# samuel-watson/glmmrMCML

Measured on AMD Instinct MI355X. Metric: MCML iters/sec x m chains (simlik evals/sec), higher is better.
Workload: dtype f64

## Files before the change

### glmmrmcml_amd/api.py

```python
import ctypes as C
from contextlib import contextmanager as _contextmanager

import numpy as np

from . import _lib

c_dp = C.POINTER(C.c_double)
c_ip = C.POINTER(C.c_int32)

REDUCE_FN = C.CFUNCTYPE(C.c_int, C.c_void_p, C.c_void_p, C.c_int)


class Problem(C.Structure):
    _fields_ = [("cov", c_ip), ("cov_rows", C.c_int), ("data", c_dp), ("data_len", C.c_int),
                ("eff_range", c_dp), ("eff_len", C.c_int), ("Z", c_dp), ("X", c_dp), ("y", c_dp),
                ("n", C.c_int), ("Q", C.c_int), ("P", C.c_int), ("family", C.c_char_p),
                ("link", C.c_char_p)]


class DevOpts(C.Structure):
    _fields_ = [("device", C.c_int), ("stream", C.c_void_p), ("rank", C.c_int), ("world", C.c_int),
                ("reduce", REDUCE_FN), ("reduce_user", C.c_void_p)]


# ... 404 lines not shown
                                                       _p(out) if rows else None, rows, C.byref(n)))
        return out

    def last_kernels(self):
        names = {-1: None, 0: "skinny", 1: "band", 2: "dlds", 3: "reg", 4: "sparse", 5: "component", 6: "exact",
                 7: "exact_component"}
        f = C.c_int(); b = C.c_int()
        _lib.check(_lib.lib().glmmr_mcml_ctx_last_kernels(self._h, C.byref(f), C.byref(b)))
        return names[f.value], names[b.value]

    def band_plan(self, chains, which="fwd"):
        keys = ("used", "nbands", "tiles", "gn", "nwg", "nred", "nslots", "paired", "nempty", "built")
        return _plan(_lib.lib().glmmr_mcml_dbg_band_plan, C.c_int, keys, self._h, {"fwd": 0, "bwd": 1}[which], int(chains),
                     bools=("used", "paired", "built"))

    def sparse_plan(self, chains):
        keys = ("active", "factored", "W", "nnz", "nnz_z", "nnz_l", "nblk", "max_blk", "long_rows", "fused", "qrows", "ncb")
        return _plan(_lib.lib().glmmr_mcml_dbg_sparse_plan, C.c_longlong, keys, self._h, int(chains),
                     bools=("active", "factored", "long_rows"))

    def set_trajectory(self, mode):
        _TRAJ.set(self, mode)

    def component_plan(self, chains):
        keys = ("requested", "feasible", "used", "ncomp", "max_vars", "max_rows", "empty_comps", "nitems", "waves_per_item",
                "cap_vars", "lds_bytes_per_workgroup")
        return _plan(_lib.lib().glmmr_mcml_dbg_component_plan, C.c_longlong, keys, self._h, int(chains),
                     bools=("requested", "feasible", "used"))

    def set_draws(self, mode):
# ... 412 lines not shown
```

### glmmrmcml_amd/csrc/band_plan.h

```cpp
#pragma once
#include "common.h"
#include <algorithm>
#include <map>
#include <memory>

namespace mcml {

constexpr int BD_BM = 80, BD_BN = 128, BD_BK = 32, BD_STAGES = 3;
constexpr int BD_A_BYTES = BD_BK * BD_BM * 8;
constexpr int BD_B_BYTES = BD_BK * BD_BN * 8;
constexpr int BD_STAGE_BYTES = BD_A_BYTES + BD_B_BYTES;
constexpr size_t BD_LDS_BYTES = (size_t)BD_STAGES * BD_STAGE_BYTES;
constexpr int BD_NA = 3, BD_NB = 4, BD_PER_TILE = BD_NA + BD_NB;
constexpr int BD_TILE_ELEMS = BD_BM * BD_BN;

struct BandItem { int band, kt0, kt1, slot; };
struct BandRed { int band, s0, s1, pad; };

struct BandPlanDev {
    int gn = 0, nwg = 0, nred = 0, nslots = 0;
    int paired = 0;
    DevBuf items, wg_ptr, red, part;
};

struct SkinnyPlan {
    int nrb = 0, nkc = 0, ldp = 0;
    DevBuf range;
    DevBuf part;
};

struct BandPlan {
    int M = 0, K = 0, nbands = 0;
    std::vector<int> kr;
    long tiles = 0;
    std::map<int, std::unique_ptr<BandPlanDev>> by_gn;
    std::unique_ptr<SkinnyPlan> skinny;

    void reset(int M_, int K_, const std::vector<int>& kr_)
    {
        M = M_; K = K_; kr = kr_; nbands = (M + BD_BM - 1) / BD_BM;
        tiles = 0;
        for (int b = 0; b < nbands; ++b) tiles += kr[2 * b + 1] - kr[2 * b];
        by_gn.clear();
        skinny.reset();
    }

    static bool decompose(const std::vector<int>& kr, int nbands, int gn, int target_wg, std::vector<BandItem>& items,
                          std::vector<int>& wg_ptr, std::vector<BandRed>& red, int& nslots)
    {
        items.clear(); wg_ptr.clear(); red.clear(); nslots = 0;
        constexpr long OVH = 3;
        const int npairs = (nbands + 1) / 2;
        if ((long)npairs * gn * 5 >= (long)target_wg * 4) {
            auto cost = [&](int b) { return 2L * (kr[2 * b + 1] - kr[2 * b]) + OVH; };
            int G = target_wg / gn; if (G > nbands) G = nbands; if (G < 1) G = 1;
            std::vector<int> order(nbands);
            for (int b = 0; b < nbands; ++b) order[b] = b;
            std::stable_sort(order.begin(), order.end(), [&](int a, int b) { return cost(a) > cost(b); });
            std::vector<long> load(G, 0);
            std::vector<std::vector<int>> group(G);
// ... 54 lines not shown
        return false;
    }

    int device_plan(int gn, hipStream_t s, BandPlanDev** out)
    {
        auto it = by_gn.find(gn);
        if (it != by_gn.end()) { *out = it->second.get(); return MCML_OK; }
        std::unique_ptr<BandPlanDev> d(new BandPlanDev());
        std::vector<BandItem> items; std::vector<int> wg_ptr; std::vector<BandRed> red; int nslots = 0;
        d->paired = decompose(kr, nbands, gn, 256, items, wg_ptr, red, nslots) ? 1 : 0;
        d->gn = gn; d->nwg = (int)wg_ptr.size() - 1; d->nred = (int)red.size(); d->nslots = nslots;
        MCML_TRY(d->items.ensure(sizeof(BandItem) * (items.size() + 1)));
        MCML_TRY(d->wg_ptr.ensure(sizeof(int) * wg_ptr.size()));
        MCML_HIP(hipMemcpyAsync(d->items.p, items.data(), sizeof(BandItem) * items.size(), hipMemcpyHostToDevice, s));
        MCML_HIP(hipMemcpyAsync(d->wg_ptr.p, wg_ptr.data(), sizeof(int) * wg_ptr.size(), hipMemcpyHostToDevice, s));
        if (nslots > 0) {
            MCML_TRY(d->red.ensure(sizeof(BandRed) * red.size()));
            MCML_HIP(hipMemcpyAsync(d->red.p, red.data(), sizeof(BandRed) * red.size(), hipMemcpyHostToDevice, s));
            MCML_TRY(d->part.ensure(sizeof(double) * (size_t)nslots * gn * BD_TILE_ELEMS));
        }
        MCML_HIP(hipStreamSynchronize(s));
        *out = d.get();
        by_gn[gn] = std::move(d);
        return MCML_OK;
    }
};

}
```

### glmmrmcml_amd/csrc/cabi.hip

```cpp
#include "entry.h"
#include "hmc_chain.h"
#include <atomic>

using namespace mcml;

struct Mode {
    int Ctx::*field;
    const char* env;
    const char* names[4];
    const char* valid;
    std::atomic<int> dflt{-1};

    int get()
    {
        if (dflt.load() < 0) {
            const char* e = getenv(env);
            int unset = -1, m = 0;
            for (int i = 1; e && names[i]; ++i) if (!strcmp(e, names[i])) m = i;
            dflt.compare_exchange_strong(unset, m);
        }
        return dflt.load();
    }
    int check(const char* fn, bool ok, int mode) const
    {
// ... 360 lines not shown
{
    return m <= 0 ? 0 : sample_shape(m, 0, chains).ncols;
}

extern "C" int glmmr_mcml_ctx_profile(glmmr_mcml_ctx* h, int enable, int reset, double* out8)
{
    MCML_REQUIRE(h, "profile: null context");
    Ctx& c = h->c;
    KernelProf& p = c.prof;
    if (out8) {
        out8[0] = p.ms[0]; out8[1] = (double)p.cnt[0]; out8[2] = p.ms[1]; out8[3] = (double)p.cnt[1];
        const double C = (double)c.hmc.C, dense = 2.0 * c.n * (double)c.Q * C;
        double ff = dense, fb = dense, kind = 0;
        if (c.sp.active) { ff = fb = 2.0 * (double)c.sp.nnz * C; kind = 2; }
        else {
            if (c.band_fwd) { ff = 2.0 * 80.0 * 32.0 * (double)c.band_fwd_tiles * C; kind = 1; }
            if (c.band_bwd) { fb = 2.0 * 80.0 * 32.0 * (double)c.band_bwd_tiles * C; kind = 1; }
        }
        out8[4] = ff; out8[5] = fb; out8[6] = dense; out8[7] = kind;
    }
    if (reset) for (int i = 0; i < 4; ++i) { p.ms[i] = 0; p.cnt[i] = 0; p.seen[i] = 0; }
    if (enable && !p.on) {
        MCML_HIP(hipSetDevice(c.device));
        while (p.ev.size() < 4096) { hipEvent_t e; if (hipEventCreate(&e) != hipSuccess) { (void)hipGetLastError(); break; } p.ev.push_back(e); }
    }
    p.on = enable != 0;
    return MCML_OK;
}

extern "C" int glmmr_mcml_ctx_profile_launches(glmmr_mcml_ctx* h, long long* fwd, long long* bwd)
{
    MCML_REQUIRE(h, "profile_launches: null context");
// ... 354 lines not shown
```

### glmmrmcml_amd/csrc/ctx.h

```cpp
#pragma once
#include "common.h"
#include "chol.h"
#include "covspec.h"
#include "band_plan.h"
#include "component_plan.h"
#include "step_ahead.h"

namespace mcml {

typedef int (*reduce_fn)(void* user, double* dev_buf, int n);

enum { KERNEL_SKINNY = 0, KERNEL_BAND = 1, KERNEL_DLDS = 2, KERNEL_REG = 3, KERNEL_SPARSE = 4, KERNEL_COMPONENT = 5,
       KERNEL_EXACT = 6,
       KERNEL_EXACT_COMPONENT = 7 };

struct StepRing {
    static constexpr int SLOTS = StepAhead::SLOTS;
    unsigned long long* h = nullptr;
    unsigned long long* d = nullptr;
    unsigned seq = 0;
    StepRing() = default;
    StepRing(const StepRing&) = delete;
    StepRing& operator=(const StepRing&) = delete;
    ~StepRing() { if (h) (void)hipHostFree(h); }
// ... 148 lines not shown
    DevBuf y;
    DevBuf y_given;
    DevBuf d_cov, d_data, d_blocks, d_rowblock;

    DevMat U;
    int mcols = 0;
    int niter = 0;
    int m_global = 0, niter_global = 0;
    DevMat ZU;
    bool zu_valid = false;

    DevMat L, ZL, ZLT;
    BandPlan plan_fwd, plan_bwd;
    DevBuf kr_scratch;
    bool band_fwd = false, band_bwd = false;
    long band_fwd_tiles = 0, band_bwd_tiles = 0;
    DevBuf xb;
    bool have_L = false;

    DevMat Dwork;
    DevBuf partials;
    DevBuf scalars;
    int* errflag() const { return reinterpret_cast<int*>(scalars.d() + 16); }
    int maxdim_large = 0;
    int n_small = 0, n_diag_rows = 0;
    DevBuf small_ids;

    int last_kernel[2] = {-1, -1};
    HmcState hmc;
    NutsState nuts;
    KernelProf prof;
// ... 77 lines not shown
```

### glmmrmcml_amd/csrc/ctx_hooks.hip

```cpp
#include "entry.h"
#include "sparse_plan.h"
#include <algorithm>

using namespace mcml;

extern "C" int glmmr_mcml_dbg_theta_log(glmmr_mcml_ctx* h, int enable, double* out, int cap_rows, int* nrows)
{
    MCML_REQUIRE(h, "theta_log: null context");
    Ctx& c = h->c;
    const int w = c.cov.npar + 1;
    const int have = (int)(c.theta_log.size() / (size_t)w);
    if (nrows) *nrows = have;
    if (out) {
        const int take = have < cap_rows ? have : cap_rows;
        memcpy(out, c.theta_log.data() + (size_t)(have - take) * w, sizeof(double) * (size_t)take * w);
        if (nrows) *nrows = take;
    }
    if (enable >= 0) { c.theta_log_on = enable != 0; if (enable) c.theta_log.clear(); }
    return MCML_OK;
}

extern "C" int glmmr_mcml_dbg_band_plan(glmmr_mcml_ctx* h, int which, int chains, int* out10)
{
    MCML_REQUIRE(h && (which == 0 || which == 1) && chains >= 1 && out10, "dbg_band_plan: bad argument");
// ... 8 lines not shown
    int nempty = 0;
    for (int b = 0; b < bp.nbands; ++b) nempty += bp.kr[2 * b] == bp.kr[2 * b + 1];
    int nwg = 0, nred = 0, nslots = 0, paired = 0, built = 0;
    auto it = bp.by_gn.find(gn);
    if (it != bp.by_gn.end()) {
        const BandPlanDev& d = *it->second;
        nwg = d.nwg; nred = d.nred; nslots = d.nslots; paired = d.paired; built = 1;
    } else if (bp.nbands > 0) {
        std::vector<BandItem> items; std::vector<int> wg_ptr; std::vector<BandRed> red;
        paired = BandPlan::decompose(bp.kr, bp.nbands, gn, 256, items, wg_ptr, red, nslots) ? 1 : 0;
        nwg = (int)wg_ptr.size() - 1; nred = (int)red.size();
    }
    const int v[10] = {(which ? c.band_bwd : c.band_fwd) ? 1 : 0, bp.nbands, (int)bp.tiles, gn, nwg, nred, nslots,
                       paired, nempty, built};
    for (int i = 0; i < 10; ++i) out10[i] = v[i];
    return MCML_OK;
}

extern "C" int glmmr_mcml_dbg_sparse_plan(glmmr_mcml_ctx* h, int chains, long long* out12)
{
    MCML_REQUIRE(h && chains >= 1 && out12, "dbg_sparse_plan: bad argument");
    const Ctx& c = h->c;
    const SparseZL& sp = c.sp;
    for (int i = 0; i < 12; ++i) out12[i] = 0;
    out12[0] = sp.active ? 1 : 0;
    out12[10] = cm_qrows(c.Q); out12[11] = cm_chain_blocks(chains);
    if (!sp.active) return MCML_OK;
    out12[1] = sp.factored ? 1 : 0; out12[2] = sp.W; out12[3] = sp.nnz; out12[4] = sp.nnz_z; out12[5] = sp.nnz_l;
    out12[6] = sp.nblk; out12[7] = sp.max_blk; out12[8] = cm_long_rows(c) ? 1 : 0; out12[9] = cm_fuse_width(c);
    return MCML_OK;
// ... 228 lines not shown
```

### glmmrmcml_amd/csrc/debug_hooks.hip

```cpp
#include "dgemm_mfma.h"
#include "dgemm_dl.h"
#include "dgemm_band.h"

using namespace mcml;

extern "C" int glmmr_mcml_dbg_dgemm(int M, int N, int K, const double* A, int lda,
                                    const double* B, int ldb, int b_nmajor,
                                    double alpha, double beta, double* C, int ldc,
                                    int lower_only, int force_tile)
{
    int ndev = 0;
    if (hipGetDeviceCount(&ndev) != hipSuccess || ndev == 0) {
        set_error("no HIP device: libglmmr_mcml_hip has no CPU fallback");
        return MCML_ENODEVICE;
    }
    hipStream_t s = nullptr;
    DevMat dA, dB, dC;
    if (force_tile == 40) {
        MCML_REQUIRE(!b_nmajor && !lower_only, "dbg_dgemm: the direct-to-LDS kernel takes a K-major B and all tiles");
        const int kpad = round_up(K, 32);
        MCML_TRY(dA.alloc(M, K, 32));
        MCML_HIP(hipMemset(dA.d(), 0, sizeof(double) * (size_t)dA.ld * dA.cols_alloc));
        MCML_HIP(hipMemcpy2D(dA.d(), sizeof(double) * dA.ld, A, sizeof(double) * lda, sizeof(double) * M, K, hipMemcpyHostToDevice));
        MCML_TRY(dB.alloc(kpad, N));
// ... 89 lines not shown
    MCML_HIP(hipEventCreate(&e0));
    MCML_HIP(hipEventCreate(&e1));
    MCML_HIP(hipEventRecord(e0, s));
    for (int i = 0; i < iters; i++) MCML_TRY(go());
    MCML_HIP(hipEventRecord(e1, s));
    MCML_HIP(hipEventSynchronize(e1));
    float ms = 0;
    MCML_HIP(hipEventElapsedTime(&ms, e0, e1));
    *ms_per_launch = ms / iters;
    (void)hipEventDestroy(e0);
    (void)hipEventDestroy(e1);
    return MCML_OK;
}

static int dbg_dgemm_band(int M, int N, int K, const double* A, int lda, const double* B, int ldb, double* C, int ldc,
                          int* tiles_executed, int form, int* whole_band);

extern "C" int glmmr_mcml_dbg_dgemm_band(int M, int N, int K, const double* A, int lda, const double* B, int ldb,
                                         double* C, int ldc, int* tiles_executed)
{
    return dbg_dgemm_band(M, N, K, A, lda, B, ldb, C, ldc, tiles_executed, BAND_FORM_AUTO, nullptr);
}

extern "C" int glmmr_mcml_dbg_dgemm_band_form(int M, int N, int K, const double* A, int lda, const double* B, int ldb,
                                              double* C, int ldc, int* tiles_executed, int form, int* whole_band)
{
    MCML_REQUIRE(form == BAND_FORM_8WAVE || form == BAND_FORM_FEED, "dbg_dgemm_band_form: form is 0 or 1");
    return dbg_dgemm_band(M, N, K, A, lda, B, ldb, C, ldc, tiles_executed, form, whole_band);
}

static int dbg_dgemm_band(int M, int N, int K, const double* A, int lda, const double* B, int ldb, double* C, int ldc,
                          int* tiles_executed, int form, int* whole_band)
{
    int ndev = 0;
    if (hipGetDeviceCount(&ndev) != hipSuccess || ndev == 0) {
        set_error("no HIP device: libglmmr_mcml_hip has no CPU fallback");
        return MCML_ENODEVICE;
    }
    MCML_REQUIRE(M > 0 && N > 0 && K > 0 && A && B && C, "dbg_dgemm_band: bad argument");
    hipStream_t s = nullptr;
    DevMat dA, dB, dC;
    MCML_TRY(dA.alloc(M, K, 32));
    MCML_HIP(hipMemset(dA.d(), 0, sizeof(double) * (size_t)dA.ld * dA.cols_alloc));
    MCML_HIP(hipMemcpy2D(dA.d(), sizeof(double) * dA.ld, A, sizeof(double) * lda, sizeof(double) * M, K, hipMemcpyHostToDevice));
    MCML_TRY(dB.alloc(round_up(K, 32), N));
    MCML_HIP(hipMemset(dB.d(), 0, sizeof(double) * (size_t)dB.ld * N));
    MCML_HIP(hipMemcpy2D(dB.d(), sizeof(double) * dB.ld, B, sizeof(double) * ldb, sizeof(double) * K, N, hipMemcpyHostToDevice));
    MCML_TRY(dC.alloc(M, N));
    MCML_HIP(hipMemset(dC.d(), 0, sizeof(double) * (size_t)dC.ld * N));
    MCML_REQUIRE(dlds_applicable(M, N, K, dA.d(), dA.ld, dA.cols_alloc, dB.d(), dB.ld), "dbg_dgemm_band: contract");
    const int nbands = (M + BD_BM - 1) / BD_BM;
    DevBuf kr;
    MCML_TRY(kr.ensure(sizeof(int) * 2 * nbands));
    hipLaunchKernelGGL(k_band_ranges, dim3(nbands), dim3(256), 0, s, dA.d(), dA.ld, M, K, kr.as<int>());
    MCML_HIP(hipGetLastError());
    std::vector<int> hk(2 * nbands);
    MCML_HIP(hipMemcpy(hk.data(), kr.p, sizeof(int) * 2 * nbands, hipMemcpyDeviceToHost));
    BandPlan plan;
    plan.reset(M, K, hk);
    if (tiles_executed) *tiles_executed = (int)plan.tiles;
    EpiAxpby epi{dC.d(), dC.ld, 1.0, 0.0};
    MCML_TRY(launch_gemm_band(s, plan, N, dA.d(), dA.ld, dB.d(), dB.ld, epi, nullptr, 0, form, whole_band));
    MCML_TRY(download_matrix(C, ldc, dC.d(), dC.ld, M, N, s));
    return MCML_OK;
}

extern "C" int glmmr_mcml_dbg_band_clocks(int M, int N, int iters, int mode, double* out3)
{
    MCML_REQUIRE(mode < 0 || !(mode & 15),
                 "dbg_band_clocks: modes 1, 2, 4 and 8 (the K loop with parts switched off) were retired by the commit "
                 "'Band HMC products: one K-loop pipeline under both kernel forms'; their findings are in DESIGN.md 5.1");
    int ndev = 0;
    if (hipGetDeviceCount(&ndev) != hipSuccess || ndev == 0) {
        set_error("no HIP device: libglmmr_mcml_hip has no CPU fallback");
// ... 6 lines not shown
    auto rnd = [&]() { x ^= x << 13; x ^= x >> 7; x ^= x << 17; return (double)(x >> 11) / 9007199254740992.0 * 2 - 1; };
    const bool cst = getenv("GLMMR_MCML_DBG_DATA") && !strcmp(getenv("GLMMR_MCML_DBG_DATA"), "const");
    const bool dec = getenv("GLMMR_MCML_DBG_DATA") && !strcmp(getenv("GLMMR_MCML_DBG_DATA"), "decay");
    for (int j = 0; j < M; ++j) for (int i = j; i < M; ++i) hA[i + (size_t)j * M] = cst ? 1.0 : dec ? rnd() * std::exp(-(double)(i - j) / 40.0) : rnd();
    for (auto& v : hB) v = cst ? 1.0 : rnd();
    DevMat dA, dB, dC;
    MCML_TRY(dA.alloc(M, M, 32));
    MCML_HIP(hipMemset(dA.d(), 0, sizeof(double) * (size_t)dA.ld * dA.cols_alloc));
    MCML_HIP(hipMemcpy2D(dA.d(), sizeof(double) * dA.ld, hA.data(), sizeof(double) * M, sizeof(double) * M, M, hipMemcpyHostToDevice));
    MCML_TRY(dB.alloc(round_up(M, 32), N));
    MCML_HIP(hipMemset(dB.d(), 0, sizeof(double) * (size_t)dB.ld * N));
    MCML_HIP(hipMemcpy2D(dB.d(), sizeof(double) * dB.ld, hB.data(), sizeof(double) * M, sizeof(double) * M, N, hipMemcpyHostToDevice));
    MCML_TRY(dC.alloc(M, N));
    const int nbands = (M + BD_BM - 1) / BD_BM;
    DevBuf kr, clk;
    MCML_TRY(kr.ensure(sizeof(int) * 2 * nbands));
    MCML_TRY(clk.ensure(16));
    MCML_HIP(hipMemset(clk.p, 0, 16));
    hipLaunchKernelGGL(k_band_ranges, dim3(nbands), dim3(256), 0, s, dA.d(), dA.ld, M, M, kr.as<int>());
    std::vector<int> hk(2 * nbands);
    MCML_HIP(hipMemcpy(hk.data(), kr.p, sizeof(int) * 2 * nbands, hipMemcpyDeviceToHost));
    BandPlan plan;
    plan.reset(M, M, hk);
    const double tiles = (double)plan.tiles;
    EpiAxpby epi{dC.d(), dC.ld, 1.0, 0.0};
    if (mode < 0) {
        for (int i = 0; i < 3; i++)
            MCML_TRY((launch_gemm_band<EpiAxpby, false>(s, plan, N, dA.d(), dA.ld, dB.d(), dB.ld, epi)));
        hipEvent_t f0, f1;
        MCML_HIP(hipEventCreate(&f0));
        MCML_HIP(hipEventCreate(&f1));
        MCML_HIP(hipEventRecord(f0, s));
        for (int i = 0; i < iters; i++)
            MCML_TRY((launch_gemm_band<EpiAxpby, false>(s, plan, N, dA.d(), dA.ld, dB.d(), dB.ld, epi)));
        MCML_HIP(hipEventRecord(f1, s));
        MCML_HIP(hipEventSynchronize(f1));
        float fms = 0;
        MCML_HIP(hipEventElapsedTime(&fms, f0, f1));
// ... 222 lines not shown
```

### glmmrmcml_amd/csrc/dgemm_band.h

```cpp
#pragma once
#include "dgemm_dlds.h"
#include "band_plan.h"

namespace mcml {

struct BandP {
    GemmP g;
    const BandItem* items;
    const int* wg_ptr;
    int nwg;
    double* part;
    int mode;
    unsigned long long* clocks;
};

static __global__ __launch_bounds__(256) void k_band_ranges(const double* A, int lda, int M, int K, int* krange)
{
    __shared__ int smin[256], smax[256];
    const int band = blockIdx.x, r0 = band * BD_BM;
    const int rows = (M - r0 < BD_BM) ? (M - r0) : BD_BM;
    int kmin = 1 << 30, kmax = -1;
    for (int k = threadIdx.x; k < K; k += 256) {
        const double* col = A + r0 + (size_t)k * lda;
        bool nz = false;
        for (int r = 0; r < rows; ++r) nz |= (col[r] != 0.0);
        if (nz) { kmin = min(kmin, k); kmax = max(kmax, k); }
    }
    smin[threadIdx.x] = kmin; smax[threadIdx.x] = kmax;
    __syncthreads();
    for (int o = 128; o > 0; o >>= 1) {
        if ((int)threadIdx.x < o) {
            smin[threadIdx.x] = min(smin[threadIdx.x], smin[threadIdx.x + o]);
            smax[threadIdx.x] = max(smax[threadIdx.x], smax[threadIdx.x + o]);
        }
        __syncthreads();
    }
    if (threadIdx.x == 0) {
        if (smax[0] < 0) { krange[2 * band] = 0; krange[2 * band + 1] = 0; }
        else { krange[2 * band] = smin[0] / BD_BK; krange[2 * band + 1] = smax[0] / BD_BK + 1; }
    }
}

#if defined(__HIP_DEVICE_COMPILE__)
#define BD_RD(dst, addr, off) asm volatile("ds_read_b64 %0, %1 offset:%2" : "=v"(dst) : "v"(addr), "i"(off))
#else
#define BD_RD(dst, addr, off) (dst = 0.0)
#endif
template <int KS, int NS>
__device__ __forceinline__ void bd_read(double (&a)[5], double (&b)[NS], unsigned aaddr, unsigned baddr)
{
    static_assert(NS == 1 || NS == 2, "one or two strips per wave");
    BD_RD(a[0], aaddr, KS * 4 * BD_BM * 8);
    BD_RD(a[1], aaddr, KS * 4 * BD_BM * 8 + 128);
    BD_RD(a[2], aaddr, KS * 4 * BD_BM * 8 + 256);
// ... 8 lines not shown
    static_assert(LEAVE == 0 || LEAVE == 5 + NS, "one substep's reads");
#if defined(__HIP_DEVICE_COMPILE__)
    if constexpr (NS == 1)
        asm volatile("s_waitcnt lgkmcnt(%[n])" : "+v"(a[0]), "+v"(a[1]), "+v"(a[2]), "+v"(a[3]), "+v"(a[4]), "+v"(b[0]) : [n] "n"(LEAVE));
    else
        asm volatile("s_waitcnt lgkmcnt(%[n])" : "+v"(a[0]), "+v"(a[1]), "+v"(a[2]), "+v"(a[3]), "+v"(a[4]), "+v"(b[0]), "+v"(b[1]) : [n] "n"(LEAVE));
#endif
}
template <int NS>
__device__ __forceinline__ void bd_mfma(d4 (&acc)[NS][5][1], const double (&a)[5], const double (&b)[NS])
{
#pragma unroll
    for (int j = 0; j < NS; ++j)
#pragma unroll
        for (int i = 0; i < 5; ++i) acc[j][i][0] = __builtin_amdgcn_mfma_f64_16x16x4f64(b[j], a[i], acc[j][i][0], 0, 0, 0);
}

__device__ __forceinline__ BandItem band_item(const BandItem* ip)
{
    BandItem item{0, 0, 0, -1};
#if defined(__HIP_DEVICE_COMPILE__)
    typedef int i4s __attribute__((ext_vector_type(4)));
    i4s raw;
    asm volatile("s_load_dwordx4 %0, %1, 0x0\n\ts_waitcnt lgkmcnt(0)" : "=&s"(raw) : "s"(ip) : "memory");
    item.band = raw.x; item.kt0 = raw.y; item.kt1 = raw.z; item.slot = raw.w;
#else
    item = *ip;
#endif
    return item;
}

template <int STRIDE, int NA, int NB>
struct BandFill {
    static constexpr int PER_TILE = NA + NB, A_CHUNKS = BD_A_BYTES / 1024;
    static_assert(STRIDE * NA >= A_CHUNKS && STRIDE * NB * 1024 == BD_B_BYTES, "the role's waves cover a stage");
    const GemmP& p;
    const BandItem* items;
    const int f, lane;
    const unsigned lds0;
    const size_t stepA;
    unsigned voa[NA], vob[NB];
    const char* sA = nullptr; const char* sB = nullptr;
    BandItem item{0, 0, 0, -1};

// ... 86 lines not shown
    extern __shared__ __attribute__((aligned(16))) double smem[];
    const unsigned lds0 = (unsigned)(size_t)(lds_ptr_t) reinterpret_cast<char*>(smem);
    const int lane = wg.lane, l15 = lane & 15, lk = lane >> 4;
    const int bj = wg.bj, n0 = bj * BD_BN, it0 = wg.it0, it1 = wg.it1;

    auto stamp = [&](int i) {
        if constexpr (DBG)
            if ((bp.mode & 16) && bp.clocks && threadIdx.x == 0)
                bp.clocks[8 + 8 * (size_t)blockIdx.x + i] = __builtin_amdgcn_s_memrealtime();
    };
    stamp(0);
    bool first_item = true;
    Fill fill(bp, piece0, lane, n0, lds0);
    bool pre = false;
    int issued = 0;
    if (it0 < it1) fill.load_item(it0);
    for (int it = it0; it < it1;) {
        const int band = fill.item.band, slot = fill.item.slot;
        const int nk = fill.item.kt1 - fill.item.kt0;

        d4 acc[NJ][5][1];
#pragma unroll
        for (int j = 0; j < NJ; ++j)
#pragma unroll
            for (int i = 0; i < 5; ++i) acc[j][i][0] = d4{0.0, 0.0, 0.0, 0.0};

        if (nk > 0) {
            const unsigned aoff = lds0 + lk * (BD_BM * 8) + l15 * 8;
            const unsigned boff = lds0 + BD_A_BYTES + (((lk >> 1) * BD_BN + strip0 * 16 + l15) << 4) + ((lk & 1) << 3);
            if (!pre) { issued = 0; for (; issued < BD_STAGES - 1 && issued < nk; ++issued) fill.issue(issued); }
            fill.wait_leave(issued - 1);
            __builtin_amdgcn_s_barrier();
            if (first_item) stamp(1);
            int st = 0;
            double ra[2][5], rb[2][NJ];
            if constexpr (NS > 0) bd_read<0>(ra[0], rb[0], aoff, boff);
            for (int kt = 0; kt < nk; ++kt) {
                if (issued < nk) {
                    int sn = st + BD_STAGES - 1; if (sn >= BD_STAGES) sn -= BD_STAGES;
                    fill.issue(sn);
                    ++issued;
                }
                const unsigned aaddr = aoff + st * BD_STAGE_BYTES, baddr = boff + st * BD_STAGE_BYTES;
                int stn = st + 1; if (stn >= BD_STAGES) stn = 0;
                if constexpr (NS > 0) {
#define BD_STEP(KS, CUR, NXT)                                   \
                    bd_read<KS + 1>(ra[NXT], rb[NXT], aaddr, baddr); \
                    bd_wait<5 + NS>(ra[CUR], rb[CUR]);               \
                    bd_mfma(acc, ra[CUR], rb[CUR]);                  \
                    __builtin_amdgcn_sched_barrier(0);
                    BD_STEP(0, 0, 1) BD_STEP(1, 1, 0) BD_STEP(2, 0, 1) BD_STEP(3, 1, 0)
                    BD_STEP(4, 0, 1) BD_STEP(5, 1, 0) BD_STEP(6, 0, 1)
#undef BD_STEP
                }
                fill.wait_leave(issued - kt - 2);
                if constexpr (NS > 0) bd_wait<0>(ra[1], rb[1]);
                __builtin_amdgcn_s_barrier();
                if constexpr (NS > 0) {
                    if (kt + 1 < nk) bd_read<0>(ra[0], rb[0], aoff + stn * BD_STAGE_BYTES, boff + stn * BD_STAGE_BYTES);
                    bd_mfma(acc, ra[1], rb[1]);
                    __builtin_amdgcn_sched_barrier(0);
                }
                st = stn;
            }
        }
        if (first_item) stamp(2);
        ++it;
        pre = false;
        if (it < it1) {
            fill.load_item(it);
            const int nkn = fill.item.kt1 - fill.item.kt0;
            if (nk > 0 && nkn > 0) {
                issued = 0;
                for (; issued < BD_STAGES - 1 && issued < nkn; ++issued) fill.issue(issued);
                pre = true;
            }
        }
        if constexpr (NS > 0) {
            if (slot < 0) {
                int elane = lane;
                if constexpr (NS > 1) asm volatile("" : "+v"(elane));
                epi(acc[0], band * BD_BM, n0 + strip0 * 16, elane, p.M, p.N, band);
                if constexpr (NS > 1) {
                    __builtin_amdgcn_sched_barrier(0);
                    epi(acc[1], band * BD_BM, n0 + strip0 * 16 + 16, elane, p.M, p.N, band);
// ... 79 lines not shown
static inline int launch_gemm_band(hipStream_t s, BandPlan& plan, int N, const double* A, int lda,
                                   const double* B, int ldb, const Epi& epi,
                                   unsigned long long* clocks = nullptr, int mode = 0, int form = BAND_FORM_AUTO,
                                   int* whole_band = nullptr)
{
    const int gn = (N + BD_BN - 1) / BD_BN;
    BandPlanDev* d = nullptr;
    MCML_TRY(plan.device_plan(gn, s, &d));
    BandP bp;
    bp.clocks = clocks;
    bp.mode = mode;
    bp.g = GemmP{plan.M, N, plan.K, A, lda, B, ldb, 0, gn, 0};
    bp.items = d->items.as<BandItem>();
    bp.wg_ptr = d->wg_ptr.as<int>();
    bp.nwg = d->nwg;
    bp.part = d->part.d();
    if (whole_band) *whole_band = d->paired;
    bool feed = false;
    if constexpr (BandFeed<Epi>::ok && !DBG) {
        feed = form == BAND_FORM_AUTO ? band_feed_enabled() : form == BAND_FORM_FEED;
        if (feed) {
            MCML_TRY(ensure_dynamic_lds(reinterpret_cast<const void*>(&dgemm_band_feed_kernel<Epi>), (int)BD_LDS_BYTES));
            hipLaunchKernelGGL((dgemm_band_feed_kernel<Epi>), dim3(d->nwg * gn), dim3(512), BD_LDS_BYTES, s, bp, epi);
        }
    }
    MCML_REQUIRE(feed || form != BAND_FORM_FEED, "launch_gemm_band: no feeder form of this instantiation");
    if (!feed) {
        MCML_TRY(ensure_dynamic_lds(reinterpret_cast<const void*>(&dgemm_band_kernel<Epi, DBG>), (int)BD_LDS_BYTES));
        hipLaunchKernelGGL((dgemm_band_kernel<Epi, DBG>), dim3(d->nwg * gn), dim3(512), BD_LDS_BYTES, s, bp, epi);
    }
// ... 10 lines not shown
```

### glmmrmcml_amd/csrc/model.hip

```cpp
#include "ctx.h"
#include "component.h"
#include "dgemm_mfma.h"
#include "dgemm_band.h"
#include "glm.h"
#include "host_linalg.h"
#include "reduce.h"
#include "vecops.h"

namespace mcml {

int model_setup(Ctx& c, const double* Z, const double* X, const double* y)
{
    const int n = c.n, Q = c.Q, P = c.P;
    MCML_TRY(upload_matrix(c.Z, Z, n, Q, n, c.stream));
    MCML_TRY(upload_matrix(c.X, X, n, P, n, c.stream));
    MCML_TRY(c.y.ensure(sizeof(double) * (size_t)pad_ld(n)));
    MCML_TRY(c.xb.ensure(sizeof(double) * (size_t)pad_ld(n)));
    MCML_HIP(hipMemsetAsync(c.y.p, 0, sizeof(double) * (size_t)pad_ld(n), c.stream));
    MCML_HIP(hipMemsetAsync(c.xb.p, 0, sizeof(double) * (size_t)pad_ld(n), c.stream));
    std::vector<double> yy(y, y + n);
    if (c.flink == 8) {
        MCML_TRY(c.y_given.ensure(sizeof(double) * (size_t)pad_ld(n)));
        MCML_TRY(copy_h2d(c.y_given.p, yy.data(), sizeof(double) * n, c.stream));
        for (auto& v : yy) v = log(v);
// ... 229 lines not shown
        MCML_TRY(c.ZL.alloc(c.n, c.Q, 32));
        MCML_TRY(c.ZLT.alloc(c.Q, c.n, 32));
        MCML_HIP(hipMemsetAsync(c.ZL.d(), 0, sizeof(double) * (size_t)c.ZL.ld * c.ZL.cols_alloc, c.stream));
        MCML_HIP(hipMemsetAsync(c.ZLT.d(), 0, sizeof(double) * (size_t)c.ZLT.ld * c.ZLT.cols_alloc, c.stream));
    }
    if (c.z_width > 0) {
        MCML_TRY(z_times(c, c.L.d(), c.L.ld, c.Q, c.ZL.d(), c.ZL.ld));
    } else {
        EpiAxpby epi{c.ZL.d(), c.ZL.ld, 1.0, 0.0};
        MCML_TRY(launch_gemm<false>(c.stream, c.n, c.Q, c.Q, c.Z.d(), c.Z.ld, c.L.d(), c.L.ld, epi));
    }
    MCML_TRY(dev_transpose(c, c.ZL.d(), c.ZL.ld, c.n, c.Q, c.ZLT.d(), c.ZLT.ld));
    c.band_fwd = c.band_bwd = false;
    const char* env = getenv("GLMMR_MCML_GEMM");
    if (!(env && (!strcmp(env, "reg") || !strcmp(env, "dlds")))) {
        auto ranges = [&](const DevMat& A, int M, int K, BandPlan& plan, bool& use, long& ntiles) -> int {
            const int nb = (M + BD_BM - 1) / BD_BM;
            MCML_TRY(c.kr_scratch.ensure(sizeof(int) * 2 * (size_t)nb));
            hipLaunchKernelGGL(k_band_ranges, dim3(nb), dim3(256), 0, c.stream, A.d(), A.ld, M, K, c.kr_scratch.as<int>());
            MCML_HIP(hipGetLastError());
            std::vector<int> h(2 * (size_t)nb);
            MCML_TRY(copy_d2h(h.data(), c.kr_scratch.p, sizeof(int) * h.size(), c.stream));
            MCML_HIP(hipStreamSynchronize(c.stream));
            if (!(plan.M == M && plan.K == K && plan.kr == h))
                plan.reset(M, K, h);
            const long dense = (long)nb * ((K + BD_BK - 1) / BD_BK);
            use = (env && !strcmp(env, "band")) || plan.tiles * 5 <= dense * 4;
            ntiles = plan.tiles;
            return MCML_OK;
        };
        MCML_TRY(ranges(c.ZL, c.n, c.Q, c.plan_fwd, c.band_fwd, c.band_fwd_tiles));
        MCML_TRY(ranges(c.ZLT, c.Q, c.n, c.plan_bwd, c.band_bwd, c.band_bwd_tiles));
    }
    return MCML_OK;
}

template <int FL>
__global__ __launch_bounds__(256) void k_loglik(const double* ZU, int ldz, int n, int ncols, const double* xb,
                                                const double* y, double var_par, int flink_rt, double* partials)
{
    const int flink = FL ? FL : flink_rt;
    __shared__ double sh[4];
    int i = blockIdx.x * 256 + threadIdx.x;
    double acc = 0;
    if (i < n) {
        const double yi = y[i], xbi = xb[i];
        for (int j = blockIdx.y; j < ncols; j += gridDim.y)
// ... 164 lines not shown
```

### include/glmmr_mcml_c.h

```cpp
#ifndef GLMMR_MCML_C_H
#define GLMMR_MCML_C_H
#include <stdint.h>

#ifdef __cplusplus
extern "C" {
#endif

#define GLMMR_MCML_OK            0
#define GLMMR_MCML_EINVAL       -1
#define GLMMR_MCML_EUNSUPPORTED -2
#define GLMMR_MCML_ENOTPD       -3
#define GLMMR_MCML_ESINGULAR    -4
#define GLMMR_MCML_EHIP         -5
#define GLMMR_MCML_ENODEVICE    -6
#define GLMMR_MCML_ENOMEM       -7

const char* glmmr_mcml_last_error(void);


typedef struct glmmr_mcml_problem {
    const int32_t* cov;
    int            cov_rows;
    const double*  data;
    int            data_len;
// ... 251 lines not shown
int glmmr_mcml_dbg_fd_hessian(glmmr_mcml_objective f, void* user, int n, const double* x, double ndeps,
                              int usebounds, const double* lower, const double* upper, double* H);
int glmmr_mcml_dbg_dgemm_bench(int M, int N, int K, int b_nmajor, int iters, int force_tile,
                               double* ms_per_launch);
int glmmr_mcml_dbg_dgemm_bench2(int M, int N, int K, int b_nmajor, int iters, int force_tile, int lower_only,
                                double beta, double* ms_per_launch);
int glmmr_mcml_dbg_dgemm_band(int M, int N, int K, const double* A, int lda, const double* B, int ldb, double* C,
                              int ldc, int* tiles_executed);
int glmmr_mcml_dbg_dgemm_band_form(int M, int N, int K, const double* A, int lda, const double* B, int ldb, double* C,
                                   int ldc, int* tiles_executed, int form, int* whole_band);
int glmmr_mcml_dbg_band_clocks(int M, int N, int iters, int mode, double* out3);

#include "glmmr_mcml_info.h"
#include "glmmr_mcml_predict.h"
#include "glmmr_mcml_sandwich.h"

#ifdef __cplusplus
}
#endif
#endif
```

Baseline: 1223.

## Skip MFMAs outside per-16-row nonzero extents in banded DGEMM

```diff
diff --git a/glmmrmcml_amd/api.py b/glmmrmcml_amd/api.py
--- a/glmmrmcml_amd/api.py
+++ b/glmmrmcml_amd/api.py
@@ -442,6 +442,15 @@
         return _plan(_lib.lib().glmmr_mcml_dbg_band_plan, C.c_int, keys, self._h, {"fwd": 0, "bwd": 1}[which], int(chains),
                      bools=("used", "paired", "built"))
 
+    def band_extents(self, which="fwd"):
+        w = {"fwd": 0, "bwd": 1}[which]
+        out3 = (C.c_longlong * 3)()
+        _lib.check(_lib.lib().glmmr_mcml_dbg_band_extents(self._h, w, None, 0, out3))
+        ext = np.zeros((int(out3[0]), 5, 2), dtype=np.int32)
+        _lib.check(_lib.lib().glmmr_mcml_dbg_band_extents(self._h, w, ext.ctypes.data_as(C.POINTER(C.c_int)),
+                                                          int(ext.size), out3))
+        return ext, int(out3[1]), int(out3[2])
+
     def sparse_plan(self, chains):
         keys = ("active", "factored", "W", "nnz", "nnz_z", "nnz_l", "nblk", "max_blk", "long_rows", "fused", "qrows", "ncb")
         return _plan(_lib.lib().glmmr_mcml_dbg_sparse_plan, C.c_longlong, keys, self._h, int(chains),
diff --git a/glmmrmcml_amd/csrc/band_plan.h b/glmmrmcml_amd/csrc/band_plan.h
--- a/glmmrmcml_amd/csrc/band_plan.h
+++ b/glmmrmcml_amd/csrc/band_plan.h
@@ -13,14 +13,52 @@
 constexpr size_t BD_LDS_BYTES = (size_t)BD_STAGES * BD_STAGE_BYTES;
 constexpr int BD_NA = 3, BD_NB = 4, BD_PER_TILE = BD_NA + BD_NB;
 constexpr int BD_TILE_ELEMS = BD_BM * BD_BN;
+constexpr int BD_RT = BD_BM / 16;
+constexpr int BD_SUB = BD_BK / 4;
+constexpr int BD_EXT = 2 * BD_RT;
 
 struct BandItem { int band, kt0, kt1, slot; };
 struct BandRed { int band, s0, s1, pad; };
+
+#if defined(__HIPCC__)
+#define BD_HD __host__ __device__
+#else
+#define BD_HD
+#endif
+BD_HD inline void band_ext_interior(const int* e, int& lo, int& hi)
+{
+    int s0 = e[0], s1 = e[1];
+    for (int i = 1; i < BD_RT; ++i) { if (e[2 * i] > s0) s0 = e[2 * i]; if (e[2 * i + 1] < s1) s1 = e[2 * i + 1]; }
+    lo = (s0 + BD_SUB - 1) / BD_SUB; hi = s1 / BD_SUB;
+}
+BD_HD inline unsigned band_ext_mask(int s0, int s1, int kt)
+{
+    int a = s0 - BD_SUB * kt, b = s1 - BD_SUB * kt;
+    a = a < 0 ? 0 : a;
+    b = b > BD_SUB ? BD_SUB : b;
+    return b > a ? ((1u << b) - 1u) & ~((1u << a) - 1u) : 0u;
+}
+inline long band_ext_issued(const int* e, int kt0, int kt1)
+{
+    long n = 0;
+    for (int i = 0; i < BD_RT; ++i) {
+        const int a = std::max(e[2 * i], BD_SUB * kt0), b = std::min(e[2 * i + 1], BD_SUB * kt1);
+        if (b > a) n += b - a;
+    }
+    return n;
+}
+
+static inline bool band_rowtiles_enabled()
+{
+    const char* e = getenv("GLMMR_MCML_BAND_ROWTILES");
+    return !(e && !strcmp(e, "0"));
+}
 
 struct BandPlanDev {
     int gn = 0, nwg = 0, nred = 0, nslots = 0;
     int paired = 0;
     DevBuf items, wg_ptr, red, part;
+    DevBuf ext;
 };
 
 struct SkinnyPlan {
@@ -32,18 +70,25 @@
 struct BandPlan {
     int M = 0, K = 0, nbands = 0;
     std::vector<int> kr;
+    std::vector<int> ext;
     long tiles = 0;
+    long mfmas = 0;
     std::map<int, std::unique_ptr<BandPlanDev>> by_gn;
     std::unique_ptr<SkinnyPlan> skinny;
 
-    void reset(int M_, int K_, const std::vector<int>& kr_)
+    void reset(int M_, int K_, const std::vector<int>& kr_, const std::vector<int>& ext_)
     {
-        M = M_; K = K_; kr = kr_; nbands = (M + BD_BM - 1) / BD_BM;
-        tiles = 0;
-        for (int b = 0; b < nbands; ++b) tiles += kr[2 * b + 1] - kr[2 * b];
+        M = M_; K = K_; kr = kr_; ext = ext_; nbands = (M + BD_BM - 1) / BD_BM;
+        tiles = 0; mfmas = 0;
+        for (int b = 0; b < nbands; ++b) {
+            tiles += kr[2 * b + 1] - kr[2 * b];
+            mfmas += band_ext_issued(ext.data() + BD_EXT * b, kr[2 * b], kr[2 * b + 1]);
+        }
         by_gn.clear();
         skinny.reset();
     }
+
+    long issued(bool rowtiles) const { return rowtiles ? mfmas : tiles * (BD_RT * BD_SUB); }
 
     static bool decompose(const std::vector<int>& kr, int nbands, int gn, int target_wg, std::vector<BandItem>& items,
                           std::vector<int>& wg_ptr, std::vector<BandRed>& red, int& nslots)
@@ -128,6 +173,8 @@
         MCML_TRY(d->wg_ptr.ensure(sizeof(int) * wg_ptr.size()));
         MCML_HIP(hipMemcpyAsync(d->items.p, items.data(), sizeof(BandItem) * items.size(), hipMemcpyHostToDevice, s));
         MCML_HIP(hipMemcpyAsync(d->wg_ptr.p, wg_ptr.data(), sizeof(int) * wg_ptr.size(), hipMemcpyHostToDevice, s));
+        MCML_TRY(d->ext.ensure(sizeof(int) * (ext.size() + 1)));
+        MCML_HIP(hipMemcpyAsync(d->ext.p, ext.data(), sizeof(int) * ext.size(), hipMemcpyHostToDevice, s));
         if (nslots > 0) {
             MCML_TRY(d->red.ensure(sizeof(BandRed) * red.size()));
             MCML_HIP(hipMemcpyAsync(d->red.p, red.data(), sizeof(BandRed) * red.size(), hipMemcpyHostToDevice, s));
diff --git a/glmmrmcml_amd/csrc/cabi.hip b/glmmrmcml_amd/csrc/cabi.hip
--- a/glmmrmcml_amd/csrc/cabi.hip
+++ b/glmmrmcml_amd/csrc/cabi.hip
@@ -398,8 +398,9 @@
         double ff = dense, fb = dense, kind = 0;
         if (c.sp.active) { ff = fb = 2.0 * (double)c.sp.nnz * C; kind = 2; }
         else {
-            if (c.band_fwd) { ff = 2.0 * 80.0 * 32.0 * (double)c.band_fwd_tiles * C; kind = 1; }
-            if (c.band_bwd) { fb = 2.0 * 80.0 * 32.0 * (double)c.band_bwd_tiles * C; kind = 1; }
+            const bool rt = band_rowtiles_enabled();
+            if (c.band_fwd) { ff = 2.0 * 16.0 * 4.0 * (double)c.plan_fwd.issued(rt) * C; kind = 1; }
+            if (c.band_bwd) { fb = 2.0 * 16.0 * 4.0 * (double)c.plan_bwd.issued(rt) * C; kind = 1; }
         }
         out8[4] = ff; out8[5] = fb; out8[6] = dense; out8[7] = kind;
     }
diff --git a/glmmrmcml_amd/csrc/ctx.h b/glmmrmcml_amd/csrc/ctx.h
--- a/glmmrmcml_amd/csrc/ctx.h
+++ b/glmmrmcml_amd/csrc/ctx.h
@@ -186,7 +186,6 @@
     BandPlan plan_fwd, plan_bwd;
     DevBuf kr_scratch;
     bool band_fwd = false, band_bwd = false;
-    long band_fwd_tiles = 0, band_bwd_tiles = 0;
     DevBuf xb;
     bool have_L = false;
 
diff --git a/glmmrmcml_amd/csrc/ctx_hooks.hip b/glmmrmcml_amd/csrc/ctx_hooks.hip
--- a/glmmrmcml_amd/csrc/ctx_hooks.hip
+++ b/glmmrmcml_amd/csrc/ctx_hooks.hip
@@ -46,6 +46,17 @@
     const int v[10] = {(which ? c.band_bwd : c.band_fwd) ? 1 : 0, bp.nbands, (int)bp.tiles, gn, nwg, nred, nslots,
                        paired, nempty, built};
     for (int i = 0; i < 10; ++i) out10[i] = v[i];
+    return MCML_OK;
+}
+
+extern "C" int glmmr_mcml_dbg_band_extents(glmmr_mcml_ctx* h, int which, int* ext, int cap, long long* out3)
+{
+    MCML_REQUIRE(h && (which == 0 || which == 1) && out3 && (ext || cap == 0), "dbg_band_extents: bad argument");
+    const Ctx& c = h->c;
+    const BandPlan& bp = which ? c.plan_bwd : c.plan_fwd;
+    const int nb = c.sp.active ? 0 : bp.nbands;
+    out3[0] = nb; out3[1] = nb ? bp.issued(true) : 0; out3[2] = nb ? bp.issued(false) : 0;
+    for (int i = 0; i < cap && i < BD_EXT * nb; ++i) ext[i] = bp.ext[i];
     return MCML_OK;
 }
 
diff --git a/glmmrmcml_amd/csrc/debug_hooks.hip b/glmmrmcml_amd/csrc/debug_hooks.hip
--- a/glmmrmcml_amd/csrc/debug_hooks.hip
+++ b/glmmrmcml_amd/csrc/debug_hooks.hip
@@ -127,23 +127,31 @@
 }
 
 static int dbg_dgemm_band(int M, int N, int K, const double* A, int lda, const double* B, int ldb, double* C, int ldc,
-                          int* tiles_executed, int form, int* whole_band);
+                          int* tiles_executed, int form, int* whole_band, int* ext_out, int ext_cap, long long* mfmas_issued);
 
 extern "C" int glmmr_mcml_dbg_dgemm_band(int M, int N, int K, const double* A, int lda, const double* B, int ldb,
                                          double* C, int ldc, int* tiles_executed)
 {
-    return dbg_dgemm_band(M, N, K, A, lda, B, ldb, C, ldc, tiles_executed, BAND_FORM_AUTO, nullptr);
+    return dbg_dgemm_band(M, N, K, A, lda, B, ldb, C, ldc, tiles_executed, BAND_FORM_AUTO, nullptr, nullptr, 0, nullptr);
 }
 
 extern "C" int glmmr_mcml_dbg_dgemm_band_form(int M, int N, int K, const double* A, int lda, const double* B, int ldb,
                                               double* C, int ldc, int* tiles_executed, int form, int* whole_band)
 {
     MCML_REQUIRE(form == BAND_FORM_8WAVE || form == BAND_FORM_FEED, "dbg_dgemm_band_form: form is 0 or 1");
-    return dbg_dgemm_band(M, N, K, A, lda, B, ldb, C, ldc, tiles_executed, form, whole_band);
+    return dbg_dgemm_band(M, N, K, A, lda, B, ldb, C, ldc, tiles_executed, form, whole_band, nullptr, 0, nullptr);
+}
+
+extern "C" int glmmr_mcml_dbg_dgemm_band_ext(int M, int N, int K, const double* A, int lda, const double* B, int ldb,
+                                             double* C, int ldc, int form, int* ext_out, int ext_cap, long long* mfmas_issued)
+{
+    MCML_REQUIRE(form == BAND_FORM_8WAVE || form == BAND_FORM_FEED, "dbg_dgemm_band_ext: form is 0 or 1");
+    MCML_REQUIRE(ext_out && mfmas_issued, "dbg_dgemm_band_ext: null argument");
+    return dbg_dgemm_band(M, N, K, A, lda, B, ldb, C, ldc, nullptr, form, nullptr, ext_out, ext_cap, mfmas_issued);
 }
 
 static int dbg_dgemm_band(int M, int N, int K, const double* A, int lda, const double* B, int ldb, double* C, int ldc,
-                          int* tiles_executed, int form, int* whole_band)
+                          int* tiles_executed, int form, int* whole_band, int* ext_out, int ext_cap, long long* mfmas_issued)
 {
     int ndev = 0;
     if (hipGetDeviceCount(&ndev) != hipSuccess || ndev == 0) {
@@ -164,13 +172,19 @@
     MCML_REQUIRE(dlds_applicable(M, N, K, dA.d(), dA.ld, dA.cols_alloc, dB.d(), dB.ld), "dbg_dgemm_band: contract");
     const int nbands = (M + BD_BM - 1) / BD_BM;
     DevBuf kr;
-    MCML_TRY(kr.ensure(sizeof(int) * 2 * nbands));
-    hipLaunchKernelGGL(k_band_ranges, dim3(nbands), dim3(256), 0, s, dA.d(), dA.ld, M, K, kr.as<int>());
+    MCML_TRY(kr.ensure(sizeof(int) * (2 + BD_EXT) * nbands));
+    hipLaunchKernelGGL(k_band_ranges, dim3(nbands), dim3(256), 0, s, dA.d(), dA.ld, M, K, kr.as<int>(), kr.as<int>() + 2 * nbands);
     MCML_HIP(hipGetLastError());
-    std::vector<int> hk(2 * nbands);
+    std::vector<int> hk(2 * nbands), he(BD_EXT * nbands);
     MCML_HIP(hipMemcpy(hk.data(), kr.p, sizeof(int) * 2 * nbands, hipMemcpyDeviceToHost));
+    MCML_HIP(hipMemcpy(he.data(), kr.as<int>() + 2 * nbands, sizeof(int) * BD_EXT * nbands, hipMemcpyDeviceToHost));
     BandPlan plan;
-    plan.reset(M, K, hk);
+    plan.reset(M, K, hk, he);
+    if (ext_out) {
+        MCML_REQUIRE(ext_cap >= BD_EXT * nbands, "dbg_dgemm_band: ext_out too small");
+        memcpy(ext_out, he.data(), sizeof(int) * he.size());
+    }
+    if (mfmas_issued) *mfmas_issued = plan.issued(band_rowtiles_enabled());
     if (tiles_executed) *tiles_executed = (int)plan.tiles;
     EpiAxpby epi{dC.d(), dC.ld, 1.0, 0.0};
     MCML_TRY(launch_gemm_band(s, plan, N, dA.d(), dA.ld, dB.d(), dB.ld, epi, nullptr, 0, form, whole_band));
@@ -207,14 +221,15 @@
     MCML_TRY(dC.alloc(M, N));
     const int nbands = (M + BD_BM - 1) / BD_BM;
     DevBuf kr, clk;
-    MCML_TRY(kr.ensure(sizeof(int) * 2 * nbands));
+    MCML_TRY(kr.ensure(sizeof(int) * (2 + BD_EXT) * nbands));
     MCML_TRY(clk.ensure(16));
     MCML_HIP(hipMemset(clk.p, 0, 16));
-    hipLaunchKernelGGL(k_band_ranges, dim3(nbands), dim3(256), 0, s, dA.d(), dA.ld, M, M, kr.as<int>());
-    std::vector<int> hk(2 * nbands);
+    hipLaunchKernelGGL(k_band_ranges, dim3(nbands), dim3(256), 0, s, dA.d(), dA.ld, M, M, kr.as<int>(), kr.as<int>() + 2 * nbands);
+    std::vector<int> hk(2 * nbands), he(BD_EXT * nbands);
     MCML_HIP(hipMemcpy(hk.data(), kr.p, sizeof(int) * 2 * nbands, hipMemcpyDeviceToHost));
+    MCML_HIP(hipMemcpy(he.data(), kr.as<int>() + 2 * nbands, sizeof(int) * BD_EXT * nbands, hipMemcpyDeviceToHost));
     BandPlan plan;
-    plan.reset(M, M, hk);
+    plan.reset(M, M, hk, he);
     const double tiles = (double)plan.tiles;
     EpiAxpby epi{dC.d(), dC.ld, 1.0, 0.0};
     if (mode < 0) {
diff --git a/glmmrmcml_amd/csrc/dgemm_band.h b/glmmrmcml_amd/csrc/dgemm_band.h
--- a/glmmrmcml_amd/csrc/dgemm_band.h
+++ b/glmmrmcml_amd/csrc/dgemm_band.h
@@ -8,36 +8,53 @@
     GemmP g;
     const BandItem* items;
     const int* wg_ptr;
+    const int* ext;
     int nwg;
     double* part;
     int mode;
     unsigned long long* clocks;
 };
 
-static __global__ __launch_bounds__(256) void k_band_ranges(const double* A, int lda, int M, int K, int* krange)
-{
-    __shared__ int smin[256], smax[256];
+static __global__ __launch_bounds__(256) void k_band_ranges(const double* A, int lda, int M, int K, int* krange, int* ext)
+{
+    __shared__ int smin[BD_RT][256], smax[BD_RT][256];
     const int band = blockIdx.x, r0 = band * BD_BM;
     const int rows = (M - r0 < BD_BM) ? (M - r0) : BD_BM;
-    int kmin = 1 << 30, kmax = -1;
+    int kmin[BD_RT], kmax[BD_RT];
+#pragma unroll
+    for (int i = 0; i < BD_RT; ++i) { kmin[i] = 1 << 30; kmax[i] = -1; }
     for (int k = threadIdx.x; k < K; k += 256) {
         const double* col = A + r0 + (size_t)k * lda;
-        bool nz = false;
-        for (int r = 0; r < rows; ++r) nz |= (col[r] != 0.0);
-        if (nz) { kmin = min(kmin, k); kmax = max(kmax, k); }
-    }
-    smin[threadIdx.x] = kmin; smax[threadIdx.x] = kmax;
+#pragma unroll
+        for (int i = 0; i < BD_RT; ++i) {
+            bool nz = false;
+            for (int r = 16 * i; r < 16 * i + 16 && r < rows; ++r) nz |= (col[r] != 0.0);
+            if (nz) { kmin[i] = min(kmin[i], k); kmax[i] = max(kmax[i], k); }
+        }
+    }
+#pragma unroll
+    for (int i = 0; i < BD_RT; ++i) { smin[i][threadIdx.x] = kmin[i]; smax[i][threadIdx.x] = kmax[i]; }
     __syncthreads();
     for (int o = 128; o > 0; o >>= 1) {
         if ((int)threadIdx.x < o) {
-            smin[threadIdx.x] = min(smin[threadIdx.x], smin[threadIdx.x + o]);
-            smax[threadIdx.x] = max(smax[threadIdx.x], smax[threadIdx.x + o]);
+#pragma unroll
+            for (int i = 0; i < BD_RT; ++i) {
+                smin[i][threadIdx.x] = min(smin[i][threadIdx.x], smin[i][threadIdx.x + o]);
+                smax[i][threadIdx.x] = max(smax[i][threadIdx.x], smax[i][threadIdx.x + o]);
+            }
         }
         __syncthreads();
     }
     if (threadIdx.x == 0) {
-        if (smax[0] < 0) { krange[2 * band] = 0; krange[2 * band + 1] = 0; }
-        else { krange[2 * band] = smin[0] / BD_BK; krange[2 * band + 1] = smax[0] / BD_BK + 1; }
+        int lo = 1 << 30, hi = -1;
+        for (int i = 0; i < BD_RT; ++i) {
+            const int a = smin[i][0], b = smax[i][0];
+            ext[BD_EXT * band + 2 * i] = b < 0 ? 0 : a / 4;
+            ext[BD_EXT * band + 2 * i + 1] = b < 0 ? 0 : b / 4 + 1;
+            lo = min(lo, a); hi = max(hi, b);
+        }
+        if (hi < 0) { krange[2 * band] = 0; krange[2 * band + 1] = 0; }
+        else { krange[2 * band] = lo / BD_BK; krange[2 * band + 1] = hi / BD_BK + 1; }
     }
 }
 
@@ -76,6 +93,18 @@
     for (int j = 0; j < NS; ++j)
 #pragma unroll
         for (int i = 0; i < 5; ++i) acc[j][i][0] = __builtin_amdgcn_mfma_f64_16x16x4f64(b[j], a[i], acc[j][i][0], 0, 0, 0);
+}
+
+template <int KS, int NS>
+__device__ __forceinline__ void bd_mfma_ext(d4 (&acc)[NS][5][1], const double (&a)[5], const double (&b)[NS], const unsigned (&m)[5])
+{
+#pragma unroll
+    for (int i = 0; i < 5; ++i)
+        if (m[i] & (1u << KS)) {
+            asm volatile("" ::: "memory");
+#pragma unroll
+            for (int j = 0; j < NS; ++j) acc[j][i][0] = __builtin_amdgcn_mfma_f64_16x16x4f64(b[j], a[i], acc[j][i][0], 0, 0, 0);
+        }
 }
 
 __device__ __forceinline__ BandItem band_item(const BandItem* ip)
@@ -90,6 +119,22 @@
     item = *ip;
 #endif
     return item;
+}
+
+__device__ __forceinline__ void band_ext_load(const int* ep, int (&e)[BD_EXT])
+{
+#if defined(__HIP_DEVICE_COMPILE__)
+    typedef int i8s __attribute__((ext_vector_type(8)));
+    typedef int i2s __attribute__((ext_vector_type(2)));
+    i8s lo; i2s hi;
+    asm volatile("s_load_dwordx8 %0, %2, 0x0\n\ts_load_dwordx2 %1, %2, 0x20\n\ts_waitcnt lgkmcnt(0)"
+                 : "=&s"(lo), "=&s"(hi) : "s"(ep) : "memory");
+#pragma unroll
+    for (int i = 0; i < 8; ++i) e[i] = lo[i];
+    e[8] = hi.x; e[9] = hi.y;
+#else
+    for (int i = 0; i < BD_EXT; ++i) e[i] = ep[i];
+#endif
 }
 
 template <int STRIDE, int NA, int NB>
@@ -206,10 +251,22 @@
     Fill fill(bp, piece0, lane, n0, lds0);
     bool pre = false;
     int issued = 0;
-    if (it0 < it1) fill.load_item(it0);
+    int ext[BD_EXT];
+    auto load_ext = [&]() {
+        if constexpr (NS > 0) {
+            if (bp.ext) band_ext_load(bp.ext + BD_EXT * fill.item.band, ext);
+            else {
+#pragma unroll
+                for (int i = 0; i < BD_RT; ++i) { ext[2 * i] = 0; ext[2 * i + 1] = 1 << 30; }
+            }
+        }
+    };
+    if (it0 < it1) { fill.load_item(it0); load_ext(); }
     for (int it = it0; it < it1;) {
         const int band = fill.item.band, slot = fill.item.slot;
-        const int nk = fill.item.kt1 - fill.item.kt0;
+        const int kt0 = fill.item.kt0, nk = fill.item.kt1 - kt0;
+        int il = 0, ih = 0;
+        if constexpr (NS > 0) { band_ext_interior(ext, il, ih); il -= kt0; ih -= kt0; }
 
         d4 acc[NJ][5][1];
 #pragma unroll
@@ -227,40 +284,62 @@
             int st = 0;
             double ra[2][5], rb[2][NJ];
             if constexpr (NS > 0) bd_read<0>(ra[0], rb[0], aoff, boff);
-            for (int kt = 0; kt < nk; ++kt) {
-                if (issued < nk) {
-                    int sn = st + BD_STAGES - 1; if (sn >= BD_STAGES) sn -= BD_STAGES;
-                    fill.issue(sn);
-                    ++issued;
-                }
-                const unsigned aaddr = aoff + st * BD_STAGE_BYTES, baddr = boff + st * BD_STAGE_BYTES;
-                int stn = st + 1; if (stn >= BD_STAGES) stn = 0;
-                if constexpr (NS > 0) {
-#define BD_STEP(KS, CUR, NXT)                                   \
+#define BD_KLOOP(LAST, BODY)                                                                         \
+            for (; kt < (LAST); ++kt) {                                                              \
+                if (issued < nk) {                                                                   \
+                    int sn = st + BD_STAGES - 1; if (sn >= BD_STAGES) sn -= BD_STAGES;               \
+                    fill.issue(sn);                                                                  \
+                    ++issued;                                                                        \
+                }                                                                                    \
+                const unsigned aaddr = aoff + st * BD_STAGE_BYTES, baddr = boff + st * BD_STAGE_BYTES; \
+                int stn = st + 1; if (stn >= BD_STAGES) stn = 0;                                     \
+                BODY                                                                                 \
+                st = stn;                                                                            \
+            }
+#define BD_STEP(KS, CUR, NXT, MFMA)                                  \
                     bd_read<KS + 1>(ra[NXT], rb[NXT], aaddr, baddr); \
                     bd_wait<5 + NS>(ra[CUR], rb[CUR]);               \
-                    bd_mfma(acc, ra[CUR], rb[CUR]);                  \
+                    MFMA(KS, CUR);                                   \
                     __builtin_amdgcn_sched_barrier(0);
-                    BD_STEP(0, 0, 1) BD_STEP(1, 1, 0) BD_STEP(2, 0, 1) BD_STEP(3, 1, 0)
-                    BD_STEP(4, 0, 1) BD_STEP(5, 1, 0) BD_STEP(6, 0, 1)
+#define BD_TILE(MFMA)                                                                                                     \
+                    BD_STEP(0, 0, 1, MFMA) BD_STEP(1, 1, 0, MFMA) BD_STEP(2, 0, 1, MFMA) BD_STEP(3, 1, 0, MFMA)           \
+                    BD_STEP(4, 0, 1, MFMA) BD_STEP(5, 1, 0, MFMA) BD_STEP(6, 0, 1, MFMA)                                  \
+                    fill.wait_leave(issued - kt - 2);                                                                     \
+                    bd_wait<0>(ra[1], rb[1]);                                                                             \
+                    __builtin_amdgcn_s_barrier();                                                                         \
+                    if (kt + 1 < nk) bd_read<0>(ra[0], rb[0], aoff + stn * BD_STAGE_BYTES, boff + stn * BD_STAGE_BYTES);  \
+                    MFMA(7, 1);                                                                                           \
+                    __builtin_amdgcn_sched_barrier(0);
+#define BD_MFMA_ALL(KS, CUR) bd_mfma(acc, ra[CUR], rb[CUR])
+#define BD_MFMA_EXT(KS, CUR) bd_mfma_ext<KS>(acc, ra[CUR], rb[CUR], em)
+#define BD_TILE_EDGE                                                                                                      \
+                    unsigned em[BD_RT];                                                                                   \
+                    _Pragma("unroll")                                                                                     \
+                    for (int i = 0; i < BD_RT; ++i) em[i] = band_ext_mask(ext[2 * i], ext[2 * i + 1], kt0 + kt);          \
+                    BD_TILE(BD_MFMA_EXT)
+            int kt = 0;
+            if constexpr (NS > 0) {
+                const int e0 = il < 0 ? 0 : (il < nk ? il : nk);
+                const int e1 = ih < e0 ? e0 : (ih < nk ? ih : nk);
+                BD_KLOOP(e0, BD_TILE_EDGE)
+                BD_KLOOP(e1, BD_TILE(BD_MFMA_ALL))
+                BD_KLOOP(nk, BD_TILE_EDGE)
+            } else {
+                BD_KLOOP(nk, fill.wait_leave(issued - kt - 2); __builtin_amdgcn_s_barrier();)
+            }
+#undef BD_TILE_EDGE
+#undef BD_MFMA_EXT
+#undef BD_MFMA_ALL
+#undef BD_TILE
 #undef BD_STEP
-                }
-                fill.wait_leave(issued - kt - 2);
-                if constexpr (NS > 0) bd_wait<0>(ra[1], rb[1]);
-                __builtin_amdgcn_s_barrier();
-                if constexpr (NS > 0) {
-                    if (kt + 1 < nk) bd_read<0>(ra[0], rb[0], aoff + stn * BD_STAGE_BYTES, boff + stn * BD_STAGE_BYTES);
-                    bd_mfma(acc, ra[1], rb[1]);
-                    __builtin_amdgcn_sched_barrier(0);
-                }
-                st = stn;
-            }
+#undef BD_KLOOP
         }
         if (first_item) stamp(2);
         ++it;
         pre = false;
         if (it < it1) {
             fill.load_item(it);
+            load_ext();
             const int nkn = fill.item.kt1 - fill.item.kt0;
             if (nk > 0 && nkn > 0) {
                 issued = 0;
@@ -370,6 +449,7 @@
     bp.items = d->items.as<BandItem>();
     bp.wg_ptr = d->wg_ptr.as<int>();
     bp.nwg = d->nwg;
+    bp.ext = band_rowtiles_enabled() ? d->ext.as<int>() : nullptr;
     bp.part = d->part.d();
     if (whole_band) *whole_band = d->paired;
     bool feed = false;
diff --git a/glmmrmcml_amd/csrc/model.hip b/glmmrmcml_amd/csrc/model.hip
--- a/glmmrmcml_amd/csrc/model.hip
+++ b/glmmrmcml_amd/csrc/model.hip
@@ -267,23 +267,24 @@
     c.band_fwd = c.band_bwd = false;
     const char* env = getenv("GLMMR_MCML_GEMM");
     if (!(env && (!strcmp(env, "reg") || !strcmp(env, "dlds")))) {
-        auto ranges = [&](const DevMat& A, int M, int K, BandPlan& plan, bool& use, long& ntiles) -> int {
+        auto ranges = [&](const DevMat& A, int M, int K, BandPlan& plan, bool& use) -> int {
             const int nb = (M + BD_BM - 1) / BD_BM;
-            MCML_TRY(c.kr_scratch.ensure(sizeof(int) * 2 * (size_t)nb));
-            hipLaunchKernelGGL(k_band_ranges, dim3(nb), dim3(256), 0, c.stream, A.d(), A.ld, M, K, c.kr_scratch.as<int>());
+            MCML_TRY(c.kr_scratch.ensure(sizeof(int) * (2 + BD_EXT) * (size_t)nb));
+            hipLaunchKernelGGL(k_band_ranges, dim3(nb), dim3(256), 0, c.stream, A.d(), A.ld, M, K, c.kr_scratch.as<int>(),
+                               c.kr_scratch.as<int>() + 2 * (size_t)nb);
             MCML_HIP(hipGetLastError());
-            std::vector<int> h(2 * (size_t)nb);
-            MCML_TRY(copy_d2h(h.data(), c.kr_scratch.p, sizeof(int) * h.size(), c.stream));
+            std::vector<int> all((2 + BD_EXT) * (size_t)nb);
+            MCML_TRY(copy_d2h(all.data(), c.kr_scratch.p, sizeof(int) * all.size(), c.stream));
             MCML_HIP(hipStreamSynchronize(c.stream));
-            if (!(plan.M == M && plan.K == K && plan.kr == h))
-                plan.reset(M, K, h);
+            const std::vector<int> h(all.begin(), all.begin() + 2 * (size_t)nb), he(all.begin() + 2 * (size_t)nb, all.end());
+            if (!(plan.M == M && plan.K == K && plan.kr == h && plan.ext == he))
+                plan.reset(M, K, h, he);
             const long dense = (long)nb * ((K + BD_BK - 1) / BD_BK);
             use = (env && !strcmp(env, "band")) || plan.tiles * 5 <= dense * 4;
-            ntiles = plan.tiles;
             return MCML_OK;
         };
-        MCML_TRY(ranges(c.ZL, c.n, c.Q, c.plan_fwd, c.band_fwd, c.band_fwd_tiles));
-        MCML_TRY(ranges(c.ZLT, c.Q, c.n, c.plan_bwd, c.band_bwd, c.band_bwd_tiles));
+        MCML_TRY(ranges(c.ZL, c.n, c.Q, c.plan_fwd, c.band_fwd));
+        MCML_TRY(ranges(c.ZLT, c.Q, c.n, c.plan_bwd, c.band_bwd));
     }
     return MCML_OK;
 }
diff --git a/include/glmmr_mcml_band.h b/include/glmmr_mcml_band.h
--- /dev/null
+++ b/include/glmmr_mcml_band.h
@@ -0,0 +1,12 @@
+#ifndef GLMMR_MCML_BAND_H
+#define GLMMR_MCML_BAND_H
+#ifndef GLMMR_MCML_C_H
+#error "include glmmr_mcml_c.h, which includes this header"
+#endif
+
+
+int glmmr_mcml_dbg_band_extents(glmmr_mcml_ctx* ctx, int which, int* ext, int cap, long long* out3);
+int glmmr_mcml_dbg_dgemm_band_ext(int M, int N, int K, const double* A, int lda, const double* B, int ldb, double* C,
+                                  int ldc, int form, int* ext_out, int ext_cap, long long* mfmas_issued);
+
+#endif
diff --git a/include/glmmr_mcml_c.h b/include/glmmr_mcml_c.h
--- a/include/glmmr_mcml_c.h
+++ b/include/glmmr_mcml_c.h
@@ -289,6 +289,7 @@
 #include "glmmr_mcml_info.h"
 #include "glmmr_mcml_predict.h"
 #include "glmmr_mcml_sandwich.h"
+#include "glmmr_mcml_band.h"
 
 #ifdef __cplusplus
 }
```

After: 1238 (median of 6 runs). +1.2%, better.
